# xingchensong/TouchNet

Hardware: AMD Instinct MI355X
Metric: audio+text tokens/sec/node (packed seq, full train step) + step MFU (higher is better)
Workload: dtype bf16

## Files before the change

touchnet_amd/_C.py:

```python
from __future__ import annotations

import ctypes as C
import os

import torch

_HERE = os.path.dirname(os.path.abspath(__file__))
LIB_PATH = os.environ.get("TN_AMD_LIB") or os.path.join(_HERE, "_lib", "libtouchnet_amd.so")

_vp, _i, _f, _ll, _ull = C.c_void_p, C.c_int, C.c_float, C.c_longlong, C.c_ulonglong

PROTOTYPES = {
    "tn_version": [],
    "tn_norm_bwd_workspace_floats": [_i, _i],
    "tn_rmsnorm_fwd": [_vp, _vp, _vp, _vp, _vp, _vp, _i, _i, _f, _i, _vp],
    "tn_rmsnorm_bwd": [_vp, _vp, _vp, _vp, _vp, _vp, _vp, _vp, _i, _i, _i, _vp],
    "tn_layernorm_fwd": [_vp, _vp, _vp, _vp, _vp, _vp, _vp, _vp, _i, _i, _f, _i, _vp],
    "tn_layernorm_bwd": [_vp, _vp, _vp, _vp, _vp, _vp, _vp, _vp, _vp, _vp, _i, _i, _i, _vp],
    "tn_swiglu_fwd": [_vp, _vp, _vp, _ll, _i, _vp],
    "tn_swiglu_bwd": [_vp, _vp, _vp, _vp, _vp, _ll, _i, _vp],
    "tn_gelu_fwd": [_vp, _vp, _ll, _i, _vp],
    "tn_gelu_bwd": [_vp, _vp, _vp, _ll, _i, _vp],
    "tn_rope_table": [_vp, _vp, _vp, _vp, _i, _i, _f, _i, _vp],
    "tn_rope_apply": [_vp, _vp, _vp, _vp, _vp, _vp, _i, _i, _i, _i, _i, _i, _vp],
# ... 36 lines not shown
    "tn_adamw_prepare": [_vp, _vp, _f, _f, _f, _vp],
    "tn_adamw_multi": [_vp, _vp, _vp, _vp, _vp, _vp, _vp, _i, _ll, _vp, _f, _f, _f, _f, _f, _i, _vp],
    "tn_adamw_multi_bounded": [_vp, _vp, _vp, _vp, _vp, _vp, _vp, _i, _ll, _vp, _f, _f, _f, _f, _f, _i, _i, _vp],
    "tn_pack_plan": [_vp, _i, _i, _i, _i, _vp, _vp, _vp, _vp, _vp, _vp],
    "tn_pack_fill": [_vp, _vp, _vp, _vp, _i, _i, _vp, _vp, _vp, _vp, _vp, _vp, _i, _i, _i, _ll, _ll, _ll, _vp, _vp, _vp,
                     _vp, _vp, _vp, _vp, _vp],
    "tn_gemm_bf16_tn": [_vp, _vp, _vp, _vp, _vp, _i, _i, _i, _ll, _ll, _ll, _ll, _i, _vp],
    "tn_gemm_bf16_addend": [_vp, _vp, _ll, _ll, _i, _i, _i, _vp, _vp, _vp, _ll, _i, _i, _ll, _vp],
    "tn_gemm_bf16_splitk": [_vp, _vp, _ll, _ll, _i, _i, _i, _vp, _vp, _i, _i, _ll, _i, _i, _i, _vp, _ll, _vp],
    "tn_gemm_bf16_wgrad_f32": [_vp, _vp, _ll, _ll, _i, _vp, _i, _i, _ll, _i, _i, _vp, _ll, _vp],
    "tn_gemm_bf16": [C.POINTER(_vp), C.POINTER(_vp), C.POINTER(_ll), C.POINTER(_ll), C.POINTER(_i), _i, _i, _i, _vp, _vp,
                     _vp, _i, _i, _ll, _ll, _i, _vp],
    "tn_gemm_splitk_workspace_bytes": [_i, _i, _i, _i, _i],
    "tn_gemm_grouped_workspace_bytes": [C.POINTER(_i), C.POINTER(_i), C.POINTER(_i), _i],
    "tn_gemm_bf16_grouped": [C.POINTER(_vp), C.POINTER(_vp), C.POINTER(_ll), C.POINTER(_ll), C.POINTER(_i), C.POINTER(_vp),
                             C.POINTER(_ll), C.POINTER(_i), C.POINTER(_i), _i, _i, _i, _i, _i, _vp, _ll, _vp],
    "tn_gemm_grouped_table_bytes": [_i],
    "tn_gemm_bf16_grouped_table": [C.POINTER(_vp), C.POINTER(_vp), C.POINTER(_ll), C.POINTER(_ll), C.POINTER(_i),
                                   C.POINTER(_vp), C.POINTER(_ll), C.POINTER(_i), C.POINTER(_i), C.POINTER(_vp), _i, _i, _i,
                                   _vp, _ll, _vp],
    "tn_gemm_bf16_wgrad_bias": [_vp, _vp, _ll, _ll, _i, _vp, _vp, _i, _i, _ll, _i, _i, _i, _vp, _ll, _vp],
    "tn_gemm_bf16_rope": [_vp, _vp, _vp, _vp, _vp, _vp, _i, _i, _i, _ll, _ll, _ll, _i, _vp],
    "tn_gemm_bf16_gelu_fwd": [_vp, _vp, _vp, _vp, _vp, _i, _i, _i, _ll, _ll, _ll, _vp],
    "tn_gemm_bf16_gelu_bwd": [_vp, _vp, _vp, _vp, _i, _i, _i, _ll, _ll, _ll, _vp],
    "tn_gemm_bf16_swiglu_fwd": [_vp, _vp, _vp, _vp, _vp, _vp, _i, _i, _i, _ll, _ll, _ll, _vp],
    "tn_gemm_bf16_swiglu_bwd": [_vp, _vp, _vp, _vp, _vp, _vp, _i, _i, _i, _ll, _ll, _ll, _vp],
    "tn_gemm_set_persistent": [_i],
    "tn_gemm_get_persistent": [],
    "tn_attn_decode_workspace_bytes": [_i, _i, _i, _i, _i],
    "tn_attn_decode": [_vp, _vp, _vp, _vp, _vp, _vp, _vp, _vp, _i, _i, _i, _i, _i, _f, _vp],
    "tn_greedy_step": [_vp, _vp, _vp, _vp, _vp, _vp, _i, _i, _i, _f, _i, _i, _i, _i, _vp],
    "tn_sample_step": [_vp, _vp, _vp, _vp, _vp, _vp, _vp, _vp, _vp, _i, _i, _i, _f, _i, _f, _i, _f, _ull, _vp, _i, _i, _i,
                       _vp],
    "tn_kimi_text_step": [_vp] * 11 + [_i, _i, _i, _i, _f, _i, _f, _i, _ull, _i, _i, _i, _i, _vp],
    "tn_attn_decode_beam": [_vp, _vp, _vp, _vp, _vp, _vp, _vp, _vp, _vp, _i, _i, _i, _i, _i, _f, _vp],
    "tn_beam_step_workspace_bytes": [_i, _i],
    "tn_beam_step": [_vp] * 17 + [_i, _i, _i, _i, _i, _f, _i, _vp, _i, _i, _f, _i, _i, _vp],
    "tn_logits_constrain": [_vp] * 13 + [_i] * 11 + [_vp],
    "tn_beam_step_edits": [_vp] * 17 + [_i, _i, _i, _i, _i, _f, _i, _vp, _i, _i, _f, _i, _i, _vp, _vp, _vp, _i, _vp],
    "tn_token_scores": [_vp] * 8 + [_i] * 5 + [_vp],
    "tn_attn_block_causal_fwd": [_vp, _vp, _vp, _vp, _vp, _vp, _i, _i, _i, _i, _i, _f, _vp],
    "tn_vq_nearest": [_vp, _vp, _vp, _vp, _i, _i, _i, _vp],
    "tn_edit_align_ws_words": [_i, _i],
    "tn_edit_align": [_vp, _ll, _vp, _ll, _vp, _vp, _i, _vp, _ll, _vp, _ll, _vp, _vp],
}
_RESTYPE = {"tn_gemm_set_persistent": None, "tn_version": C.c_char_p, "tn_sumsq_multi_chunk": C.c_longlong, "tn_adamw_multi_chunk": C.c_longlong,
            "tn_colsum_workspace_floats": C.c_longlong, "tn_gemm_splitk_workspace_bytes": C.c_longlong,
            "tn_gemm_grouped_workspace_bytes": C.c_longlong, "tn_gemm_grouped_table_bytes": C.c_longlong,
            "tn_attn_decode_workspace_bytes": C.c_longlong, "tn_beam_step_workspace_bytes": C.c_longlong,
            "tn_edit_align_ws_words": C.c_longlong, "tn_philox4x32_10": None}

DEV_PROTOTYPES = {
    "tn_philox4x32_10": [_vp, _ull],
}

_lib = None


class KernelError(RuntimeError):
    pass


def lib() -> C.CDLL:
    global _lib
    if _lib is None:
        if not os.path.exists(LIB_PATH):
            raise ImportError(
                f"{LIB_PATH} not found: build it with `python -m touchnet_amd.build` "
                "(touchnet_amd has no fallback path; the HIP extension is mandatory)")
        handle = C.CDLL(LIB_PATH)
        for name, argtypes in {**PROTOTYPES, **DEV_PROTOTYPES}.items():
            fn = getattr(handle, name)
            fn.argtypes = argtypes
            fn.restype = _RESTYPE.get(name, C.c_int)
        _lib = handle
    return _lib


def check(code: int, what: str) -> None:
    if code != 0:
        raise KernelError(f"{what} failed with code {code} "
                          f"({'EINVAL: unsupported shape/dtype' if code == -22 else 'hipError_t'})")


DTYPE_CODE = {torch.float32: 0, torch.bfloat16: 1}


def dcode(t: torch.Tensor) -> int:
    try:
        return DTYPE_CODE[t.dtype]
    except KeyError:
        raise KernelError(f"unsupported dtype {t.dtype} (float32 / bfloat16 only)") from None


def ptr(t):
    if t is None:
        return None
    if not t.is_cuda:
        raise KernelError("touchnet_amd kernels need device (HIP) tensors; got a CPU tensor")
    return C.c_void_p(t.data_ptr())


def stream():
    return C.c_void_p(torch.cuda.current_stream().cuda_stream)


# ... 3 lines not shown
```

touchnet_amd/csrc/gemm.hip:

```cpp
#include "gemm_host.h"

namespace tn {
namespace gemm {

typedef f32x4_t Acc16[8][4];

template <bool AK, bool BK, int EPI = EPI_PLAIN>
struct Kernel16 {
  static_assert(EPI == EPI_PLAIN || EPI == EPI_SWIGLU_FWD || EPI == EPI_SWIGLU_BWD || EPI == EPI_ROPE ||
                    EPI == EPI_GELU_FWD || EPI == EPI_GELU_BWD,
                "Kernel16: plain / SwiGLU / RoPE / GELU epilogues (the weight-gradient modes stay on Kernel)");
  static_assert(EPI != EPI_GELU_FWD || !BK, "GELU forward: x W^T layout");
  static_assert(EPI != EPI_GELU_BWD || BK, "GELU backward: dY W layout");
  static_assert(!AK, "Kernel16: row-stored A (forward and input-gradient products)");
  static_assert(EPI != EPI_SWIGLU_FWD || !BK, "SwiGLU forward: x W^T layout");
  static_assert(EPI != EPI_SWIGLU_BWD || BK, "SwiGLU backward: dY W layout");
  static_assert(EPI != EPI_ROPE || !BK, "RoPE epilogue: x W^T layout");
  static constexpr int BN_EFF = EPI == EPI_SWIGLU_FWD ? 128 : BN;
  static __device__ __forceinline__ float sigm(float x) { return sigmoid_fast(x); }
  static __device__ __forceinline__ float lo16(uint32_t w) { return __uint_as_float(w << 16); }
  static __device__ __forceinline__ float hi16(uint32_t w) { return __uint_as_float(w & 0xffff0000u); }
  static __device__ __forceinline__ float rbf(float v) { return __uint_as_float(((uint32_t)f2bf(v)) << 16); }
  template <bool KMAJ>
  struct F4 {
// ... 1 lines not shown
    u32x2_t h[KMAJ ? 4 : 1][2];
  };
  template <bool KMAJ, int NB >
  struct Reader {
    int x[KMAJ ? NB / 2 : 2];
    __device__ __forceinline__ Reader(int lane, int row0) {
      const int l15 = lane & 15, g4 = lane >> 4;
      if constexpr (!KMAJ) {
        const int f = (l15 >> 1) & 7;
#pragma unroll
        for (int h = 0; h < 2; ++h) x[h] = (row0 + l15) * 128 + (((4 * h + g4) ^ f) << 4);
      } else {
        const int j = l15 >> 2, w = l15 & 3;
#pragma unroll
        for (int g = 0; g < NB / 2; ++g)
          x[g] = (8 * g4 + j) * 512 + w * 8 + ((((row0 >> 5) + g) ^ j) << 6) + (g4 & 1) * 32;
      }
    }
    template <int H, int BLK, int I>
    __device__ __forceinline__ void read(const char* smem, int sbase, F4<KMAJ>& f) const {
      if constexpr (!KMAJ) {
        f.v[I] = __builtin_bit_cast(bf16x8_t, *reinterpret_cast<const u32x4_t*>(smem + sbase + x[H] + BLK * 2048));
      } else {
        const uint32_t a = (uint32_t)(size_t)(lds_ptr_t)smem + (uint32_t)(sbase + (x[BLK >> 1] ^ ((BLK & 1) * 32)));
        f.h[I][0] = ds_tr16<(32 * H) * 512>(a);
        f.h[I][1] = ds_tr16<(32 * H + 4) * 512>(a);
      }
    }
  };
  template <bool KMAJ>
  static __device__ __forceinline__ void retire(F4<KMAJ>& f) {
    if constexpr (KMAJ) {
      asm volatile("s_waitcnt lgkmcnt(0)"
                   : "+v"(f.h[0][0]), "+v"(f.h[0][1]), "+v"(f.h[1][0]), "+v"(f.h[1][1]), "+v"(f.h[2][0]), "+v"(f.h[2][1]),
                     "+v"(f.h[3][0]), "+v"(f.h[3][1]));
#pragma unroll
      for (int i = 0; i < 4; ++i) {
        const u32x4_t t = {f.h[i][0].x, f.h[i][0].y, f.h[i][1].x, f.h[i][1].y};
        f.v[i] = __builtin_bit_cast(bf16x8_t, t);
      }
    }
  }

  static __device__ __forceinline__ void run(const Params& p, char* smem) {
    const int tid = threadIdx.x;
    int lane = tid & 63;
    const int wave = __builtin_amdgcn_readfirstlane(tid >> 6);
    const int wr = wave >> 2, wc = wave & 3;
    const int bid = blockIdx.x, G = gridDim.x;
    const int tiles = p.ntiles;
    const int mine = (tiles - bid + G - 1) / G;
    auto origin = [&](int k, int& m0, int& n0) {
      int tm, tn;
      tile_of_block(p.tile0 + bid + k * G, p.nbm, p.nbn, tm, tn);
      m0 = tm * BM;
      n0 = tn * BN_EFF;
    };
    Stream<AK, true> sA;
    Stream<BK, true> sB;
    int ka = 0, kb = 0;
    auto open_a = [&](int s) {
      int m0, n0;
      origin(ka, m0, n0);
      sA.open(p.seg[s].A, p.seg[s].lda, p.seg[s].K, p.M, m0, wave, lane);
      sA.seg = s;
    };
    const bool b_wave0 = EPI == EPI_SWIGLU_FWD || (EPI == EPI_ROPE && p.rope_d == 128);
    auto open_b = [&](int s) {
      int m0, n0;
      origin(kb, m0, n0);
      if constexpr (EPI == EPI_SWIGLU_FWD) {
        sB.open((wave & 1) ? p.seg[1].B : p.seg[0].B, p.seg[0].ldb, p.seg[0].K, p.N, n0 + (wave >> 1) * 32, 0, lane);
      } else if constexpr (EPI == EPI_ROPE) {
        if (p.rope_d == 128)
          sB.open(p.seg[0].B, p.seg[0].ldb, p.seg[0].K, p.N, n0 + (wave >> 2) * 128 + (wave & 1) * 64 + ((wave >> 1) & 1) * 32,
                  0, lane);
        else
          sB.open(p.seg[0].B, p.seg[0].ldb, p.seg[0].K, p.N, n0, wave, lane);
      } else {
        sB.open(p.seg[s].B, p.seg[s].ldb, p.seg[s].K, p.N, n0, wave, lane);
      }
      sB.seg = s;
    };
    auto adv_a = [&]() {
      sA.soff += sA.step;
      if (--sA.left == 0) {
        if (sA.seg + 1 < p.nseg) open_a(sA.seg + 1);
        else if (++ka < mine) open_a(0);
        else sA.kill(p.C);
      }
    };
    auto adv_b = [&]() {
      sB.soff += sB.step;
      if (--sB.left == 0) {
        if (sB.seg + 1 < p.nseg) open_b(sB.seg + 1);
        else if (++kb < mine) open_b(0);
        else sB.kill(p.C);
      }
    };
    auto piece_a = [&](int slot, int q) {
      __builtin_amdgcn_raw_ptr_buffer_load_lds(sA.rs, (lds_ptr_t)(smem + slot * SLOT + wave * 4096 + q * 1024), 16,
                                               sA.voff[q], sA.soff, 0, 0);
    };
    auto piece_b = [&](int slot, int q) {
      __builtin_amdgcn_raw_ptr_buffer_load_lds(sB.rs, (lds_ptr_t)(smem + slot * SLOT + wave * 4096 + q * 1024), 16,
                                               sB.voff[q], sB.soff, 0, 0);
    };
// ... 629 lines not shown
  if (c.addend != nullptr && (c.accumulate || c.splitk > 1 || c.tail_only || c.Ct != nullptr || c.c_f32 ||
                              c.bias_grad != nullptr || !out_ok(c.addend, c.ldadd, N, 8)))
    return TN_EINVAL;
  if ((c.bias_grad != nullptr || c.c_f32) && (!wgrad_mode || c.tail_only)) return TN_EINVAL;
  if (!aligned(1, c.bias_grad)) return TN_EINVAL;
  if (M <= 0 || N <= 0 || c.nseg < 1 || c.nseg > MAXSEG || (N % 8) != 0 || (c.a_kmaj && (M % 8))) return TN_EINVAL;
  if (!out_ok(c.C, c.ldc, N, 8)) return TN_EINVAL;
  if (c.Ct != nullptr && ((M % 8) || c.accumulate || !out_ok(c.Ct, c.ldct, M, 8))) return TN_EINVAL;
  Params p;
  clear_params(p);
  for (int s = 0; s < c.nseg; ++s) {
    const int k = c.K[s];
    if (!(c.a_kmaj ? kmaj_operand_ok(c.A[s], c.lda[s], k, M, M) : row_operand_ok(c.A[s], c.lda[s], k, 1))) return TN_EINVAL;
    if (!(c.b_kmaj ? kmaj_operand_ok(c.B[s], c.ldb[s], k, N, 1) : row_operand_ok(c.B[s], c.ldb[s], k, 1))) return TN_EINVAL;
    set_seg(p.seg[s], c.A[s], c.B[s], c.lda[s], c.ldb[s], k);
    p.stages += (k + 63) / 64;
  }
  for (int s = c.nseg; s < MAXSEG; ++s) p.seg[s] = p.seg[0];
  p.nseg = c.nseg;
  p.M = M;
  p.N = N;
  p.C = (bf16_t*)c.C;
  p.Ct = (bf16_t*)c.Ct;
  p.bias = (const bf16_t*)c.bias;
  p.ldc = c.ldc;
  p.ldct = c.ldct;
  p.accumulate = c.accumulate;
  p.addend = (const bf16_t*)c.addend;
  p.ldadd = c.ldadd;
  p.nbm = (M + BM - 1) / BM;
  p.nbn = (N + BN - 1) / BN;
  p.ntiles = p.nbm * p.nbn;
  p.c_f32 = c.c_f32;
  p.bias_out = (bf16_t*)c.bias_grad;
  const int ncu = num_cus();
  int main_tiles = 0;
  if (c.splitk > 1) {
    if (c.nseg != 1 || c.Ct != nullptr) return TN_EINVAL;
    if (!(c.a_kmaj && c.b_kmaj) && (p.stages % c.splitk) != 0) return TN_EINVAL;
    const long long need = tn_gemm_splitk_workspace_bytes(M, N, c.splitk, c.bias_grad != nullptr, c.tail_only);
    if (need < 0 || c.workspace == nullptr || !aligned(15, c.workspace) || c.workspace_bytes < need) return TN_EINVAL;
    if (c.tail_only) main_tiles = p.ntiles / ncu * ncu;
    p.splitk = c.splitk;
    p.kchunk = (p.stages + c.splitk - 1) / c.splitk;
    p.ws = (float*)c.workspace;
    if (c.bias_grad != nullptr) p.bias_ws = p.ws + slab_floats(c.splitk, p.ntiles);
  }
  hipStream_t st = (hipStream_t)c.stream;
  int rc = 0;
  if (main_tiles > 0) {
    Params pm = p;
    pm.splitk = 1;
    pm.ntiles = main_tiles;
    rc |= launch_mode(c.a_kmaj, c.b_kmaj, c.Ct != nullptr, dim3(ncu), st, pm);
    p.tile0 = main_tiles;
    p.ntiles -= main_tiles;
  }
  rc |= launch_mode(c.a_kmaj, c.b_kmaj, c.Ct != nullptr, grid_for(p.ntiles * p.splitk), st, p);
  if (rc != 0) return TN_EINVAL;
  TN_LAUNCH_CHECK();
  return TN_OK;
}

template <int EPI, bool B_KMAJ>
int launch_fused(Params& p, int M, int N, long long ldc, int col_tile, void* stream) {
  for (int s = 1; s < MAXSEG; ++s)
    if (p.seg[s].K == 0) p.seg[s] = p.seg[0];
  p.stages = p.seg[0].K / 64;
  p.M = M;
  p.N = N;
  p.ldc = ldc;
  p.nbm = (M + BM - 1) / BM;
  p.nbn = (N + col_tile - 1) / col_tile;
  p.ntiles = p.nbm * p.nbn;
  hipLaunchKernelGGL((gemm16_kernel<false, B_KMAJ, EPI>), grid_for(p.ntiles), dim3(NT), 0, (hipStream_t)stream, p);
  TN_LAUNCH_CHECK();
  return TN_OK;
}

}

extern "C" {

void tn_gemm_set_persistent(int on) { g_persistent = on ? 1 : 0; }
int tn_gemm_get_persistent(void) { return g_persistent; }

long long tn_gemm_splitk_workspace_bytes(int M, int N, int splitk, int with_bias_grad, int tail_only) {
  if (splitk <= 1) return 0;
  if (M <= 0 || N <= 0) return -1;
  const long long nbm = (M + BM - 1) / BM;
  long long tiles = nbm * ((N + BN - 1) / BN);
  if (tail_only) {
    const int ncu = num_cus();
    if (tiles < ncu || tiles % ncu == 0) return -1;
    tiles %= ncu;
  }
  return (slab_floats(splitk, tiles) + (with_bias_grad ? splitk * nbm * BM : 0)) * (long long)sizeof(float);
}

int tn_gemm_bf16(const void* const* A, const void* const* B, const long long* lda, const long long* ldb, const int* K,
                 int nseg, int a_kmaj, int b_kmaj, void* C, void* Ct, const void* bias, int M, int N, long long ldc,
                 long long ldct, int accumulate, void* stream) {
  GemmCall c{A, B, lda, ldb, K, nseg, a_kmaj, b_kmaj, C, ldc, M, N, stream};
  c.bias = bias;
  c.accumulate = accumulate;
  c.Ct = Ct;
  c.ldct = ldct;
  return gemm_launch(c);
}

int tn_gemm_bf16_addend(const void* A, const void* B, long long lda, long long ldb, int K, int a_kmaj, int b_kmaj, void* C,
                        const void* bias, const void* addend, long long ldadd, int M, int N, long long ldc, void* stream) {
  if (addend == nullptr || addend == C) return TN_EINVAL;
  GemmCall c{&A, &B, &lda, &ldb, &K, 1, a_kmaj, b_kmaj, C, ldc, M, N, stream};
  c.bias = bias;
  c.addend = addend;
  c.ldadd = ldadd;
  return gemm_launch(c);
}

int tn_gemm_bf16_splitk(const void* A, const void* B, long long lda, long long ldb, int K, int a_kmaj, int b_kmaj,
                        void* C, const void* bias, int M, int N, long long ldc, int accumulate, int splitk, int tail_only,
                        void* workspace, long long workspace_bytes, void* stream) {
  if (splitk < 2) return TN_EINVAL;
  GemmCall c{&A, &B, &lda, &ldb, &K, 1, a_kmaj, b_kmaj, C, ldc, M, N, stream};
  c.bias = bias;
  c.accumulate = accumulate;
  c.splitk = splitk;
  c.tail_only = tail_only;
  c.workspace = workspace;
  c.workspace_bytes = workspace_bytes;
  return gemm_launch(c);
}

static int wgrad(const void* A, const void* B, long long lda, long long ldb, int K, void* C, void* bias_grad, int M, int N,
                 long long ldc, int accumulate, int c_f32, int splitk, void* workspace, long long workspace_bytes,
                 void* stream) {
  GemmCall c{&A, &B, &lda, &ldb, &K, 1, 1, 1, C, ldc, M, N, stream};
// ... 12 lines not shown
  return wgrad(A, B, lda, ldb, K, C, nullptr, M, N, ldc, accumulate, 1, splitk, workspace, workspace_bytes, stream);
}

int tn_gemm_bf16_wgrad_bias(const void* A, const void* B, long long lda, long long ldb, int K, void* C, void* bias_grad,
                            int M, int N, long long ldc, int accumulate, int c_f32, int splitk, void* workspace,
                            long long workspace_bytes, void* stream) {
  if (bias_grad == nullptr) return TN_EINVAL;
  return wgrad(A, B, lda, ldb, K, C, bias_grad, M, N, ldc, accumulate, c_f32, splitk, workspace, workspace_bytes, stream);
}

long long tn_gemm_grouped_workspace_bytes(const int* M, const int* N, const int* K, int ngrp) {
  if (ngrp < 1 || ngrp > MAXSEG) return -1;
  long long tiles = 0;
  int min_stages = 0x7fffffff, r;
  for (int g = 0; g < ngrp; ++g) {
    tiles += (long long)((M[g] + BM - 1) / BM) * ((N[g] + BN - 1) / BN);
    min_stages = min(min_stages, (K[g] + 63) / 64);
  }
  const int S = grouped_split(tiles, min_stages, r);
  return S > 1 ? slab_floats(S, r) * (long long)sizeof(float) : 0;
}

int tn_gemm_bf16_grouped(const void* const* A, const void* const* B, const long long* lda, const long long* ldb,
                         const int* K, void* const* C, const long long* ldc, const int* M, const int* N, int ngrp,
                         int a_kmaj, int b_kmaj, int accumulate, int c_f32, void* workspace, long long workspace_bytes,
                         void* stream) {
  if (ngrp < 1 || ngrp > MAXSEG) return TN_EINVAL;
  if (!(a_kmaj && b_kmaj)) return TN_EINVAL;
  Params p;
  clear_params(p);
  int total = 0, min_stages = 0x7fffffff;
  for (int g = 0; g < ngrp; ++g) {
    if (!grouped_product(A[g], B[g], lda[g], ldb[g], K[g], C[g], ldc[g], M[g], N[g], c_f32, total, p.seg[g], p.grp[g]))
      return TN_EINVAL;
    min_stages = min(min_stages, p.grp[g].stages);
    total += p.grp[g].nbm * p.grp[g].nbn;
  }
  for (int g = ngrp; g < MAXSEG; ++g) {
    p.seg[g] = p.seg[0];
    p.grp[g] = p.grp[0];
    p.grp[g].start = 0x7fffffff;
  }
  p.ngrp = ngrp;
  p.accumulate = accumulate;
  p.c_f32 = c_f32;
  hipStream_t st = (hipStream_t)stream;
  int r, S = grouped_split(total, min_stages, r);
  if (S > 1 && (workspace == nullptr || !aligned(15, workspace) ||
                workspace_bytes < slab_floats(S, r) * (long long)sizeof(float)))
    S = 1;
  const int main_tiles = S > 1 ? total - r : total;
  p.tile0 = 0;
  p.ntiles = main_tiles;
  if (c_f32)
    hipLaunchKernelGGL((gemm_kernel<true, true, false, false, true, EPI_GROUPED>), grid_for(main_tiles), dim3(NT), 0, st, p);
  else
    hipLaunchKernelGGL((gemm_kernel<true, true, false, false, false, EPI_GROUPED>), grid_for(main_tiles), dim3(NT), 0, st, p);
  if (S > 1) {
    float* ws = (float*)workspace;
    for (int g = 0; g < ngrp; ++g) {
      const int end = p.grp[g].start + p.grp[g].nbm * p.grp[g].nbn;
      const int lo = max(main_tiles, p.grp[g].start), hi = end;
      if (lo >= hi) continue;
      Params q;
      clear_params(q);
      q.seg[0] = p.seg[g];
      q.seg[1] = q.seg[2] = q.seg[0];
      q.M = p.grp[g].M;
      q.N = p.grp[g].N;
      q.C = p.grp[g].C;
      q.ldc = p.grp[g].ldc;
      q.accumulate = accumulate;
      q.nbm = p.grp[g].nbm;
      q.nbn = p.grp[g].nbn;
      q.stages = p.grp[g].stages;
      q.splitk = S;
      q.kchunk = (q.stages + S - 1) / S;
      q.ws = ws;
      q.tile0 = lo - p.grp[g].start;
      q.ntiles = hi - lo;
      q.c_f32 = c_f32;
      hipLaunchKernelGGL((gemm_kernel<true, true, false, true>), grid_for(q.ntiles * S), dim3(NT), 0, st, q);
      hipLaunchKernelGGL(splitk_reduce_kernel, dim3((unsigned)q.ntiles * 32u), dim3(256), 0, st, q.ws, q.splitk, q.M, q.N,
                         q.nbm, q.nbn, q.tile0, q.ntiles, q.C, q.ldc, (const bf16_t*)nullptr, q.accumulate, q.c_f32,
                         (const float*)nullptr, (bf16_t*)nullptr);
      ws += slab_floats(S, q.ntiles);
    }
  }
  TN_LAUNCH_CHECK();
  return TN_OK;
}
int tn_gemm_bf16_swiglu_fwd(const void* x, const void* wg, const void* wu, void* gate, void* up, void* act, int M, int I,
                            int K, long long ldx, long long ldw, long long ldc, void* stream) {
  if (M <= 0 || I <= 0 || (I % 8) || !row_operand_ok(x, ldx, K, K) || !row_operand_ok(wg, ldw, K, K) ||
      !row_operand_ok(wu, ldw, K, K) || !out_ok(gate, ldc, I, 8) || !aligned(15, up, act))
    return TN_EINVAL;
  Params p;
  clear_params(p);
  set_seg(p.seg[0], x, wg, ldx, ldw, K);
  set_seg(p.seg[1], x, wu, ldx, ldw, K);
  p.C = (bf16_t*)gate;
  p.C2 = (bf16_t*)up;
  p.C3 = (bf16_t*)act;
  return launch_fused<EPI_SWIGLU_FWD, false>(p, M, I, ldc, 128, stream);
}

// ... 69 lines not shown
```

touchnet_amd/csrc/gemm_host.h:

```cpp
#pragma once

#include "gemm_kernel.h"

using namespace tn::gemm;
using tn::bf16_t;

extern "C" int tn_gemm_get_persistent(void);

namespace {

int num_cus() {
  static const int ncu = [] {
    int dev = 0, n = 256;
    if (hipGetDevice(&dev) == hipSuccess) (void)hipDeviceGetAttribute(&n, hipDeviceAttributeMultiprocessorCount, dev);
    return n >= 8 ? n / 8 * 8 : 8;
  }();
  return ncu;
}

bool persistent_now() {
  const char* pe = getenv("TN_GEMM_PERSIST");
  return pe ? atoi(pe) != 0 : tn_gemm_get_persistent() != 0;
}

dim3 grid_for(int units) {
  const int ncu = num_cus();
  return dim3(persistent_now() && units > ncu ? ncu : units);
}

void clear_params(Params& p) {
  p = Params{};
  p.splitk = 1;
  p.nseg = 1;
}

void set_seg(Seg& s, const void* A, const void* B, long long lda, long long ldb, int K) {
  s.A = (const bf16_t*)A;
  s.B = (const bf16_t*)B;
  s.lda = lda;
  s.ldb = ldb;
  s.K = K;
  s.pad_ = 0;
}

template <typename... P>
bool aligned(uintptr_t mask, P... ps) {
  return ((... | (uintptr_t)ps) & mask) == 0;
}

constexpr long long DMA_SPAN = 0x7fffffffLL;

bool row_operand_ok(const void* X, long long ld, int K, long long min_ld) {
  return K > 0 && (K % 64) == 0 && aligned(15, X) && (ld % 8) == 0 && ld >= min_ld && 288 * ld * 2 < DMA_SPAN;
}

bool kmaj_operand_ok(const void* X, long long ld, int K, int rows, long long min_ld) {
  return K > 0 && aligned(15, X) && (ld % 8) == 0 && ld >= min_ld && ((long long)(K - 1) * ld + rows) * 2 < DMA_SPAN;
}

bool out_ok(const void* C, long long ld, int cols, int ld_mult) { return aligned(15, C) && (ld % ld_mult) == 0 && ld >= cols; }

bool grouped_product(const void* A, const void* B, long long lda, long long ldb, int k, void* C, long long ldc, int m, int n,
                     int c_f32, int start, Seg& s, Grp& g) {
  if (m <= 0 || n <= 0 || (m % 8) || (n % 8) || !kmaj_operand_ok(A, lda, k, m, m) || !kmaj_operand_ok(B, ldb, k, n, 1) ||
      !out_ok(C, ldc, n, c_f32 ? 4 : 8))
    return false;
  set_seg(s, A, B, lda, ldb, k);
  g.C = (bf16_t*)C;
  g.ldc = ldc;
  g.M = m;
  g.N = n;
  g.nbm = (m + BM - 1) / BM;
  g.nbn = (n + BN - 1) / BN;
  g.start = start;
  g.stages = (k + 63) / 64;
  return true;
}

}
```

touchnet_amd/csrc/gemm_kernel.h:

```cpp
#pragma once

#include <stdlib.h>

#include <type_traits>
#include <utility>
#include <vector>

#include "common.h"

namespace tn {
namespace gemm {

constexpr int BM = 256, BN = 256;
constexpr int SLOT = 32768;
constexpr int LDS_BYTES = 5 * SLOT;
constexpr int NT = 512;
constexpr int MAXSEG = 3;

typedef __attribute__((address_space(3))) void* lds_ptr_t;
typedef __attribute__((ext_vector_type(2))) uint32_t u32x2_t;
typedef __attribute__((ext_vector_type(4))) uint32_t u32x4_t;

struct Seg {
  const bf16_t* A;
  const bf16_t* B;
  long long lda, ldb;
  int K;
  int pad_;
};

struct Grp {
  bf16_t* C;
  long long ldc;
  int M, N, nbm, nbn;
  int start;
  int stages;
};

struct Rec {
  Seg seg;
  Grp grp;
  bf16_t* bias_out;
};
typedef const __attribute__((address_space(4))) Rec* rec_ptr_t;
constexpr int MAXTAB = 1024;
constexpr int TABCHUNK = 32;

constexpr int EPI_PLAIN = 0, EPI_GROUPED = 1, EPI_SWIGLU_FWD = 2, EPI_SWIGLU_BWD = 3, EPI_BIASG = 4, EPI_ROPE = 5;
constexpr int EPI_GELU_FWD = 6, EPI_GELU_BWD = 7, EPI_TABLE = 8;

struct Params {
  Seg seg[MAXSEG];
  int nseg;
  int M, N;
  bf16_t* C;
  bf16_t* Ct;
  const bf16_t* bias;
  long long ldc, ldct;
  int accumulate;
  const bf16_t* addend;
  long long ldadd;
  int nbm, nbn;
  int stages;
  int splitk, kchunk;
  float* ws;
  int tile0, ntiles;
  int c_f32;
  Grp grp[MAXSEG];
  int ngrp;
  bf16_t* C2;
  bf16_t* C3;
  const bf16_t* E1;
  const bf16_t* E2;
  long long lde;
  bf16_t* bias_out;
  float* bias_ws;
  const bf16_t* rope_cos;
  const bf16_t* rope_sin;
  int rope_d;
  const Rec* table;
};

__device__ __forceinline__ int xcd_chunk(int bid, int total) {
  const int xcd = bid & 7, local = bid >> 3;
  const int q = total >> 3, r = total & 7;
  return (xcd < r ? xcd * (q + 1) : r * (q + 1) + (xcd - r) * q) + local;
}

__device__ __forceinline__ void panel_group(int vid, int nbm, int nbn, int& tm, int& tn) {
  constexpr int GM = 8;
  const int per_group = GM * nbn;
  const int g = vid / per_group, w = vid - g * per_group;
  const int gm = min(GM, nbm - g * GM);
  tm = g * GM + w % gm;
  tn = w / gm;
}

__device__ __forceinline__ void tile_of_block(int bid, int nbm, int nbn, int& tm, int& tn) {
  panel_group(xcd_chunk(bid, nbm * nbn), nbm, nbn, tm, tn);
}

typedef f32x16_t Acc[4][2];

constexpr int kPieceB[4] = {0, 2, 4, 6}, kPieceA[4] = {14, 18, 22, 26};
static_assert(kPieceB[3] < kPieceA[0], "every B piece is issued before the first A piece");

template <bool IS_A> constexpr int piece_at(int pos) {
  for (int i = 0; i < 4; ++i)
    if ((IS_A ? kPieceA[i] : kPieceB[i]) == pos) return i;
  return -1;
}
constexpr int early_piece_count() {
  int n = 0;
  for (int i = 0; i < 4; ++i) n += (kPieceB[i] < 8) + (kPieceA[i] < 8);
  return n;
}

template <bool KMAJ, bool M16 = false>
struct Stream {
  __amdgpu_buffer_rsrc_t rs;
  int soff;
  int step;
  int left;
  int seg;
  int ld2;
  int voff[4];

  __device__ __forceinline__ void set_voff(int wave, int lane) {
    if constexpr (!KMAJ) {
#pragma unroll
      for (int q = 0; q < 4; ++q) {
        const int row = wave * 32 + q * 8 + (lane >> 3);
        voff[q] = row * ld2 + (((lane & 7) ^ ((row >> 1) & 7)) << 4);
      }
    } else {
#pragma unroll
      for (int q = 0; q < 4; ++q) {
        const int k = wave * 8 + q * 2 + (lane >> 5);
        const int u = lane & 31;
        const int ch = M16 ? ((u & 3) ^ (((k >> 3) & 1) << 1)) : (u & 3);
        voff[q] = k * ld2 + ((((u >> 2) ^ (k & 3)) << 6) | (ch << 4));
      }
    }
  }

  __device__ __forceinline__ void open(const bf16_t* X, long long ld, int K, int R, int origin, int wave, int lane) {
    ld2 = (int)(ld * 2);
    if constexpr (!KMAJ) {
      const long long bytes = R > origin ? (long long)(R - origin - 1) * ld2 + 2LL * K : 0LL;
      rs = __builtin_amdgcn_make_buffer_rsrc((void*)(X + (long long)origin * ld), 0, (int)min(bytes, 0x7fffffffLL),
                                             0x00020000);
      step = 128;
    } else {
// ... 90 lines not shown
#pragma unroll
      for (int j = 0; j < 2; ++j) {
        const u32x4_t t = {b.h[j][0].x, b.h[j][0].y, b.h[j][1].x, b.h[j][1].y};
        b.v[j] = __builtin_bit_cast(bf16x8_t, t);
      }
    }
  }

  static __device__ __forceinline__ void run(const Params& p, char* smem) { body(p, smem); }

  static __device__ __forceinline__ void body(const Params& p, char* smem) {
    const int tid = threadIdx.x;
    int lane = tid & 63;
    const int wave = __builtin_amdgcn_readfirstlane(tid >> 6);
    const int wr = wave >> 2, wc = wave & 3;

    const int bid = blockIdx.x, G = gridDim.x;
    const int tiles = p.ntiles;
    const int mine = ((SPLITK ? tiles * p.splitk : tiles) - bid + G - 1) / G;
    const rec_ptr_t tab = (rec_ptr_t)p.table;
    auto seg_of = [&](int g) {
      if constexpr (EPI == EPI_TABLE) {
        Seg s;
        s.A = tab[g].seg.A;
        s.B = tab[g].seg.B;
        s.lda = tab[g].seg.lda;
        s.ldb = tab[g].seg.ldb;
        s.K = tab[g].seg.K;
        s.pad_ = 0;
        return s;
      } else {
        return p.seg[g];
      }
    };
    auto grp_of = [&](int g) {
      if constexpr (EPI == EPI_TABLE) {
        Grp r;
        r.C = tab[g].grp.C;
        r.ldc = tab[g].grp.ldc;
        r.M = tab[g].grp.M;
        r.N = tab[g].grp.N;
        r.nbm = tab[g].grp.nbm;
        r.nbn = tab[g].grp.nbn;
        r.start = tab[g].grp.start;
        r.stages = tab[g].grp.stages;
        return r;
      } else {
        return p.grp[g];
      }
    };
    auto origin_g = [&](int k, int& m0, int& n0, int& g) {
      int tm, tn, u = bid + k * G;
      if constexpr (SPLITK) u -= (u / tiles) * tiles;
      u += p.tile0;
      g = 0;
      if constexpr (EPI == EPI_TABLE) {
        u = xcd_chunk(u, tiles);
        int hi = p.ngrp - 1;
        while (g < hi) {
          const int mid = (g + hi + 1) >> 1;
          if (tab[mid].grp.start <= u) g = mid;
          else hi = mid - 1;
        }
      } else if constexpr (EPI == EPI_GROUPED) {
        if (p.ngrp > 1 && u >= p.grp[1].start) g = 1;
        if (p.ngrp > 2 && u >= p.grp[2].start) g = 2;
      }
      if constexpr (EPI == EPI_TABLE) {
        const Grp r = grp_of(g);
        panel_group(u - r.start, r.nbm, r.nbn, tm, tn);
      } else if constexpr (EPI == EPI_GROUPED) {
        const Grp r = grp_of(g);
        tile_of_block(u - r.start, r.nbm, r.nbn, tm, tn);
      } else {
        tile_of_block(u, p.nbm, p.nbn, tm, tn);
      }
      m0 = tm * BM;
      n0 = tn * BN;
    };
    auto origin = [&](int k, int& m0, int& n0) {
      int g;
      origin_g(k, m0, n0, g);
    };
    auto split_of = [&](int k) { return (bid + k * G) / tiles; };

    Stream<AK> sA;
    Stream<BK> sB;
    int ka = 0, kb = 0;
    auto open_a = [&](int s) {
      int m0, n0;
      origin(ka, m0, n0);
      if constexpr (SPLITK) {
        const int k0 = split_of(ka) * p.kchunk * 64, klen = min(p.seg[0].K - k0, p.kchunk * 64);
        if (klen > 0) sA.open(p.seg[0].A + (AK ? (long long)k0 * p.seg[0].lda : (long long)k0), p.seg[0].lda, klen, p.M,
                              m0, wave, lane);
        else sA.kill(p.C);
        sA.left = p.kchunk;
      } else if constexpr (MULTI) {
        int g;
        origin_g(ka, m0, n0, g);
        const Seg sg = seg_of(g);
        sA.open(sg.A, sg.lda, sg.K, grp_of(g).M, m0, wave, lane);
      } else {
        sA.open(p.seg[s].A, p.seg[s].lda, p.seg[s].K, p.M, m0, wave, lane);
      }
      sA.seg = s;
    };
    auto open_b = [&](int s) {
      int m0, n0;
      origin(kb, m0, n0);
      if constexpr (SPLITK) {
        const int k0 = split_of(kb) * p.kchunk * 64, klen = min(p.seg[0].K - k0, p.kchunk * 64);
        if (klen > 0) sB.open(p.seg[0].B + (BK ? (long long)k0 * p.seg[0].ldb : (long long)k0), p.seg[0].ldb, klen, p.N,
                              n0, wave, lane);
        else sB.kill(p.C);
        sB.left = p.kchunk;
      } else if constexpr (MULTI) {
        int g;
        origin_g(kb, m0, n0, g);
        const Seg sg = seg_of(g);
        sB.open(sg.B, sg.ldb, sg.K, grp_of(g).N, n0, wave, lane);
      } else {
        sB.open(p.seg[s].B, p.seg[s].ldb, p.seg[s].K, p.N, n0, wave, lane);
      }
      sB.seg = s;
    };
    auto adv_a = [&]() {
      sA.soff += sA.step;
// ... 397 lines not shown
```

touchnet_amd/csrc/gemm_table.hip:

```cpp
#include "gemm_host.h"

namespace tn {
namespace gemm {

struct RecChunk {
  Rec r[TABCHUNK];
};
static_assert(sizeof(Rec) % 8 == 0 && sizeof(RecChunk) <= 3072, "a chunk of records fits the kernel-argument segment");
constexpr int REC_WORDS = (int)(sizeof(Rec) / 8);

__global__ __launch_bounds__(TABCHUNK * REC_WORDS) void table_upload_kernel(const RecChunk c, Rec* dst, int n) {
  const int t = threadIdx.x;
  if (t < n * REC_WORDS)
    reinterpret_cast<unsigned long long*>(dst)[t] = reinterpret_cast<const unsigned long long*>(&c)[t];
}

}
}

extern "C" {

long long tn_gemm_grouped_table_bytes(int n) { return n < 1 || n > MAXTAB ? -1 : (long long)n * (long long)sizeof(Rec); }

int tn_gemm_bf16_grouped_table(const void* const* A, const void* const* B, const long long* lda, const long long* ldb,
                               const int* K, void* const* C, const long long* ldc, const int* M, const int* N,
                               void* const* bias_grad, int n, int accumulate, int c_f32, void* table, long long table_bytes,
                               void* stream) {
  if (n < 1 || n > MAXTAB) return TN_EINVAL;
  if (table == nullptr || !aligned(15, table) || table_bytes < tn_gemm_grouped_table_bytes(n)) return TN_EINVAL;
  std::vector<RecChunk> chunks((n + TABCHUNK - 1) / TABCHUNK);
  long long total = 0;
  for (int g = 0; g < n; ++g) {
    Rec& r = chunks[g / TABCHUNK].r[g % TABCHUNK];
    if (total > 0x7fffffff) return TN_EINVAL;
    if (!grouped_product(A[g], B[g], lda[g], ldb[g], K[g], C[g], ldc[g], M[g], N[g], c_f32, (int)total, r.seg, r.grp))
      return TN_EINVAL;
    r.bias_out = bias_grad != nullptr ? (bf16_t*)bias_grad[g] : nullptr;
    if (!aligned(1, r.bias_out)) return TN_EINVAL;
    total += (long long)r.grp.nbm * r.grp.nbn;
  }
  if (total > 0x7fffffff) return TN_EINVAL;
  hipStream_t st = (hipStream_t)stream;
  for (int c = 0; c * TABCHUNK < n; ++c)
    hipLaunchKernelGGL(table_upload_kernel, dim3(1), dim3(TABCHUNK * REC_WORDS), 0, st, chunks[c],
                       (Rec*)table + c * TABCHUNK, min(TABCHUNK, n - c * TABCHUNK));
  Params p;
  clear_params(p);
  p.table = (const Rec*)table;
  p.ngrp = n;
  p.accumulate = accumulate;
  p.c_f32 = c_f32;
  p.ntiles = (int)total;
  if (c_f32)
    hipLaunchKernelGGL((gemm_kernel<true, true, false, false, true, EPI_TABLE>), grid_for(p.ntiles), dim3(NT), 0, st, p);
  else
    hipLaunchKernelGGL((gemm_kernel<true, true, false, false, false, EPI_TABLE>), grid_for(p.ntiles), dim3(NT), 0, st, p);
  TN_LAUNCH_CHECK();
  return TN_OK;
}

}
```

Baseline: 23640.

## Add host-chosen window/serpentine tile order to improve per-XCD L2 panel reuse

Adds a tile-mapping module with a second ordering, round-based windows over CUs with serpentine column-strip walks. The host simulates panel fetches per XCD for both orders, picks the one with fewer distinct row/column panels, and caches the choice by shape. All GEMM kernels (plain, Kernel16, grouped, table) now map tile indices through this shared function. The aim is more A/B panel reuse within each XCD's L2. The cost is extra index arithmetic, including an inverse-mapping loop for partial launches, and a host-side mutex and map lookup on every launch.

```diff
diff --git a/touchnet_amd/_C.py b/touchnet_amd/_C.py
--- a/touchnet_amd/_C.py
+++ b/touchnet_amd/_C.py
@@ -112,6 +112,7 @@
 
 DEV_PROTOTYPES = {
     "tn_philox4x32_10": [_vp, _ull],
+    "tn_gemm_tilemap_units": [C.POINTER(_i), C.POINTER(_i), _i, _i, _i, _i, _i, _i, _i, _i, C.POINTER(_i)],
 }
 
 _lib = None
diff --git a/touchnet_amd/csrc/gemm.hip b/touchnet_amd/csrc/gemm.hip
--- a/touchnet_amd/csrc/gemm.hip
+++ b/touchnet_amd/csrc/gemm.hip
@@ -77,7 +77,8 @@
     const int mine = (tiles - bid + G - 1) / G;
     auto origin = [&](int k, int& m0, int& n0) {
       int tm, tn;
-      tile_of_block(p.tile0 + bid + k * G, p.nbm, p.nbn, tm, tn);
+      const tilemap::List L = {1, p.total, 0, tiles, p.round, p.order, 0};
+      tilemap::tile_of_unit(bid + k * G, L, p.nbm, p.nbn, tm, tn);
       m0 = tm * BM;
       n0 = tn * BN_EFF;
     };
@@ -813,10 +814,12 @@
     Params pm = p;
     pm.splitk = 1;
     pm.ntiles = main_tiles;
+    set_tile_order(pm, p.nbm * p.nbn);
     rc |= launch_mode(c.a_kmaj, c.b_kmaj, c.Ct != nullptr, dim3(ncu), st, pm);
     p.tile0 = main_tiles;
     p.ntiles -= main_tiles;
   }
+  if (p.splitk == 1) set_tile_order(p, p.ntiles);
   rc |= launch_mode(c.a_kmaj, c.b_kmaj, c.Ct != nullptr, grid_for(p.ntiles * p.splitk), st, p);
   if (rc != 0) return TN_EINVAL;
   TN_LAUNCH_CHECK();
@@ -834,6 +837,7 @@
   p.nbm = (M + BM - 1) / BM;
   p.nbn = (N + col_tile - 1) / col_tile;
   p.ntiles = p.nbm * p.nbn;
+  set_tile_order(p, p.ntiles);
   hipLaunchKernelGGL((gemm16_kernel<false, B_KMAJ, EPI>), grid_for(p.ntiles), dim3(NT), 0, (hipStream_t)stream, p);
   TN_LAUNCH_CHECK();
   return TN_OK;
@@ -845,6 +849,37 @@
 
 void tn_gemm_set_persistent(int on) { g_persistent = on ? 1 : 0; }
 int tn_gemm_get_persistent(void) { return g_persistent; }
+
+int tn_gemm_tilemap_units(const int* nbm, const int* nbn, int ngrp, int whole, int tile0, int ntiles, int round, int order,
+                          int unit0, int count, int* out) {
+  if (ngrp < 1 || nbm == nullptr || nbn == nullptr || out == nullptr) return TN_EINVAL;
+  std::vector<int> shapes, starts;
+  long long total = 0;
+  for (int g = 0; g < ngrp; ++g) {
+    if (nbm[g] < 1 || nbn[g] < 1) return TN_EINVAL;
+    starts.push_back((int)total);
+    shapes.insert(shapes.end(), {nbm[g], nbn[g]});
+    total += (long long)nbm[g] * nbn[g];
+    if (total > 0x7fffffff) return TN_EINVAL;
+  }
+  if (tile0 < 0 || ntiles < 1 || (long long)tile0 + ntiles > total || round < 8 || (round % 8) != 0) return TN_EINVAL;
+  if (whole && (tile0 != 0 || ntiles != total)) return TN_EINVAL;
+  if (unit0 < 0 || count < 0 || (long long)unit0 + count > ntiles) return TN_EINVAL;
+  if (order < 0) order = tile0 != 0 ? tilemap::ORDER_CHUNK : tile_order((int)total, ntiles, round, whole, shapes);
+  if ((order != tilemap::ORDER_CHUNK && order != tilemap::ORDER_WINDOW) || (order == tilemap::ORDER_WINDOW && tile0 != 0))
+    return TN_EINVAL;
+  const tilemap::List L = {ngrp, (int)total, tile0, ntiles, round, order, whole};
+  for (int i = 0; i < count; ++i)
+    tilemap::tile_of_unit(
+        unit0 + i, L, [&](int pos) { return tilemap::product_at(pos, ngrp, [&](int g) { return starts[g]; }); },
+        [&](int g) { return starts[g]; },
+        [&](int g, int& m, int& n) {
+          m = shapes[2 * g];
+          n = shapes[2 * g + 1];
+        },
+        out[3 * i], out[3 * i + 1], out[3 * i + 2]);
+  return order;
+}
 
 long long tn_gemm_splitk_workspace_bytes(int M, int N, int splitk, int with_bias_grad, int tail_only) {
   if (splitk <= 1) return 0;
@@ -963,6 +998,7 @@
   const int main_tiles = S > 1 ? total - r : total;
   p.tile0 = 0;
   p.ntiles = main_tiles;
+  set_tile_order(p, total);
   if (c_f32)
     hipLaunchKernelGGL((gemm_kernel<true, true, false, false, true, EPI_GROUPED>), grid_for(main_tiles), dim3(NT), 0, st, p);
   else
diff --git a/touchnet_amd/csrc/gemm_host.h b/touchnet_amd/csrc/gemm_host.h
--- a/touchnet_amd/csrc/gemm_host.h
+++ b/touchnet_amd/csrc/gemm_host.h
@@ -1,4 +1,8 @@
 #pragma once
+
+#include <map>
+#include <mutex>
+#include <vector>
 
 #include "gemm_kernel.h"
 
@@ -32,6 +36,40 @@
   p = Params{};
   p.splitk = 1;
   p.nseg = 1;
+}
+
+int tile_order(int total, int ntiles, int round, int whole, const std::vector<int>& shapes) {
+  if (whole) return tilemap::ORDER_CHUNK;
+  static std::mutex mu;
+  static std::map<std::vector<int>, int> known;
+  std::vector<int> key = {total, ntiles, round, whole};
+  key.insert(key.end(), shapes.begin(), shapes.end());
+  std::lock_guard<std::mutex> lock(mu);
+  auto it = known.find(key);
+  if (it != known.end()) return it->second;
+  const int n = (int)shapes.size() / 2;
+  std::vector<int> starts(n, 0);
+  for (int g = 1; g < n; ++g) starts[g] = starts[g - 1] + shapes[2 * g - 2] * shapes[2 * g - 1];
+  const tilemap::List L = {n, total, 0, ntiles, round, tilemap::ORDER_CHUNK, whole};
+  const int order = tilemap::choose_order(
+      L, [&](int g) { return starts[g]; },
+      [&](int g, int& nbm, int& nbn) {
+        nbm = shapes[2 * g];
+        nbn = shapes[2 * g + 1];
+      });
+  known.emplace(std::move(key), order);
+  return order;
+}
+
+void set_tile_order(Params& p, int total) {
+  std::vector<int> shapes;
+  if (p.ngrp > 0)
+    for (int g = 0; g < p.ngrp; ++g) shapes.insert(shapes.end(), {p.grp[g].nbm, p.grp[g].nbn});
+  else
+    shapes = {p.nbm, p.nbn};
+  p.total = total;
+  p.round = num_cus();
+  p.order = tile_order(total, p.ntiles, p.round, 0, shapes);
 }
 
 void set_seg(Seg& s, const void* A, const void* B, long long lda, long long ldb, int K) {
diff --git a/touchnet_amd/csrc/gemm_kernel.h b/touchnet_amd/csrc/gemm_kernel.h
--- a/touchnet_amd/csrc/gemm_kernel.h
+++ b/touchnet_amd/csrc/gemm_kernel.h
@@ -7,6 +7,7 @@
 #include <vector>
 
 #include "common.h"
+#include "gemm_tilemap.h"
 
 namespace tn {
 namespace gemm {
@@ -65,6 +66,7 @@
   int splitk, kchunk;
   float* ws;
   int tile0, ntiles;
+  int total, round, order;
   int c_f32;
   Grp grp[MAXSEG];
   int ngrp;
@@ -81,24 +83,7 @@
   const Rec* table;
 };
 
-__device__ __forceinline__ int xcd_chunk(int bid, int total) {
-  const int xcd = bid & 7, local = bid >> 3;
-  const int q = total >> 3, r = total & 7;
-  return (xcd < r ? xcd * (q + 1) : r * (q + 1) + (xcd - r) * q) + local;
-}
-
-__device__ __forceinline__ void panel_group(int vid, int nbm, int nbn, int& tm, int& tn) {
-  constexpr int GM = 8;
-  const int per_group = GM * nbn;
-  const int g = vid / per_group, w = vid - g * per_group;
-  const int gm = min(GM, nbm - g * GM);
-  tm = g * GM + w % gm;
-  tn = w / gm;
-}
-
-__device__ __forceinline__ void tile_of_block(int bid, int nbm, int nbn, int& tm, int& tn) {
-  panel_group(xcd_chunk(bid, nbm * nbn), nbm, nbn, tm, tn);
-}
+using tilemap::tile_of_block;
 
 typedef f32x16_t Acc[4][2];
 
@@ -295,28 +280,30 @@
     auto origin_g = [&](int k, int& m0, int& n0, int& g) {
       int tm, tn, u = bid + k * G;
       if constexpr (SPLITK) u -= (u / tiles) * tiles;
-      u += p.tile0;
-      g = 0;
+      const tilemap::List L = {MULTI ? p.ngrp : 1, EPI == EPI_TABLE ? tiles : p.total, p.tile0, tiles, p.round,
+                               SPLITK || EPI == EPI_TABLE ? tilemap::ORDER_CHUNK : p.order, EPI == EPI_TABLE};
       if constexpr (EPI == EPI_TABLE) {
-        u = xcd_chunk(u, tiles);
-        int hi = p.ngrp - 1;
-        while (g < hi) {
-          const int mid = (g + hi + 1) >> 1;
-          if (tab[mid].grp.start <= u) g = mid;
-          else hi = mid - 1;
-        }
+        auto start_of = [&](int i) { return tab[i].grp.start; };
+        tilemap::tile_of_unit(
+            u, L, [&](int pos) { return tilemap::product_at(pos, p.ngrp, start_of); }, start_of,
+            [&](int i, int& nbm, int& nbn) {
+              nbm = tab[i].grp.nbm;
+              nbn = tab[i].grp.nbn;
+            },
+            g, tm, tn);
       } else if constexpr (EPI == EPI_GROUPED) {
-        if (p.ngrp > 1 && u >= p.grp[1].start) g = 1;
-        if (p.ngrp > 2 && u >= p.grp[2].start) g = 2;
-      }
-      if constexpr (EPI == EPI_TABLE) {
-        const Grp r = grp_of(g);
-        panel_group(u - r.start, r.nbm, r.nbn, tm, tn);
-      } else if constexpr (EPI == EPI_GROUPED) {
-        const Grp r = grp_of(g);
-        tile_of_block(u - r.start, r.nbm, r.nbn, tm, tn);
-      } else {
-        tile_of_block(u, p.nbm, p.nbn, tm, tn);
+        auto pick = [&](int i, int Grp::*f) { return i == 0 ? p.grp[0].*f : i == 1 ? p.grp[1].*f : p.grp[2].*f; };
+        tilemap::tile_of_unit(
+            u, L, [&](int pos) { return (int)(p.ngrp > 1 && pos >= p.grp[1].start) + (int)(p.ngrp > 2 && pos >= p.grp[2].start); },
+            [&](int i) { return pick(i, &Grp::start); },
+            [&](int i, int& nbm, int& nbn) {
+              nbm = pick(i, &Grp::nbm);
+              nbn = pick(i, &Grp::nbn);
+            },
+            g, tm, tn);
+      } else {
+        g = 0;
+        tilemap::tile_of_unit(u, L, p.nbm, p.nbn, tm, tn);
       }
       m0 = tm * BM;
       n0 = tn * BN;
diff --git a/touchnet_amd/csrc/gemm_table.hip b/touchnet_amd/csrc/gemm_table.hip
--- a/touchnet_amd/csrc/gemm_table.hip
+++ b/touchnet_amd/csrc/gemm_table.hip
@@ -51,6 +51,9 @@
   p.accumulate = accumulate;
   p.c_f32 = c_f32;
   p.ntiles = (int)total;
+  p.total = p.ntiles;
+  p.round = num_cus();
+  p.order = tile_order(p.total, p.ntiles, p.round, 1, {});
   if (c_f32)
     hipLaunchKernelGGL((gemm_kernel<true, true, false, false, true, EPI_TABLE>), grid_for(p.ntiles), dim3(NT), 0, st, p);
   else
diff --git a/touchnet_amd/csrc/gemm_tilemap.h b/touchnet_amd/csrc/gemm_tilemap.h
--- /dev/null
+++ b/touchnet_amd/csrc/gemm_tilemap.h
@@ -0,0 +1,156 @@
+#pragma once
+
+#include <algorithm>
+#include <vector>
+
+namespace tn {
+namespace gemm {
+namespace tilemap {
+
+#define TN_TILEMAP_FN __host__ __device__ __forceinline__
+
+constexpr int ORDER_CHUNK = 0, ORDER_WINDOW = 1;
+constexpr int GM = 8;
+constexpr int SW = 4;
+
+struct List {
+  int ngrp;
+  int total;
+  int tile0;
+  int ntiles;
+  int round;
+  int order;
+  int whole;
+};
+
+TN_TILEMAP_FN int xcd_chunk(int bid, int total) {
+  const int xcd = bid & 7, local = bid >> 3;
+  const int q = total >> 3, r = total & 7;
+  return (xcd < r ? xcd * (q + 1) : r * (q + 1) + (xcd - r) * q) + local;
+}
+
+TN_TILEMAP_FN int xcd_chunk_inv(int pos, int total) {
+  const int q = total >> 3, r = total & 7;
+  const int b = r * (q + 1);
+  int xcd, local;
+  if (pos < b) {
+    xcd = pos / (q + 1);
+    local = pos - xcd * (q + 1);
+  } else {
+    xcd = (pos - b) / q;
+    local = pos - b - xcd * q;
+    xcd += r;
+  }
+  return local * 8 + xcd;
+}
+
+TN_TILEMAP_FN void panel_group(int vid, int nbm, int nbn, int& tm, int& tn) {
+  const int per_group = GM * nbn;
+  const int g = vid / per_group, w = vid - g * per_group;
+  const int gm = min(GM, nbm - g * GM);
+  tm = g * GM + w % gm;
+  tn = w / gm;
+}
+
+TN_TILEMAP_FN int panel_group_inv(int tm, int tn, int nbm, int nbn) {
+  const int g = tm / GM;
+  const int gm = min(GM, nbm - g * GM);
+  return g * GM * nbn + tn * gm + (tm - g * GM);
+}
+
+TN_TILEMAP_FN int window_pos(int u, int n, int round) {
+  const int base = u / round * round;
+  return base + xcd_chunk(u - base, min(round, n - base));
+}
+
+TN_TILEMAP_FN void strip_walk(int i, int nbm, int nbn, int& tm, int& tn) {
+  const int last = max(nbn / SW, 1) - 1;
+  const int per = SW * nbm;
+  const int s = min(i / per, last);
+  const int j = i - s * per;
+  const int w = s == last ? nbn - s * SW : SW;
+  const int row = j / w;
+  tm = (s & 1) ? nbm - 1 - row : row;
+  tn = s * SW + (j - row * w);
+}
+
+template <typename StartOf>
+TN_TILEMAP_FN int product_at(int pos, int ngrp, StartOf start_of) {
+  int g = 0, hi = ngrp - 1;
+  while (g < hi) {
+    const int mid = (g + hi + 1) >> 1;
+    if (start_of(mid) <= pos) g = mid;
+    else hi = mid - 1;
+  }
+  return g;
+}
+
+template <typename Find, typename StartOf, typename ShapeOf>
+TN_TILEMAP_FN void tile_of_unit(int u, const List& L, Find find, StartOf start_of, ShapeOf shape_of, int& g, int& tm,
+                                int& tn) {
+  int nbm, nbn;
+  if (L.order == ORDER_CHUNK) {
+    u += L.tile0;
+    if (L.whole) u = xcd_chunk(u, L.total);
+    g = find(u);
+    shape_of(g, nbm, nbn);
+    u -= start_of(g);
+    panel_group(L.whole ? u : xcd_chunk(u, nbm * nbn), nbm, nbn, tm, tn);
+    return;
+  }
+  for (;;) {
+    const int v = u < L.ntiles ? window_pos(u, L.ntiles, L.round) : u;
+    g = find(v);
+    shape_of(g, nbm, nbn);
+    strip_walk(v - start_of(g), nbm, nbn, tm, tn);
+    if (L.ntiles == L.total) return;
+    u = start_of(g) + xcd_chunk_inv(panel_group_inv(tm, tn, nbm, nbn), nbm * nbn);
+    if (u < L.ntiles) return;
+  }
+}
+
+TN_TILEMAP_FN void tile_of_unit(int u, const List& L, int nbm, int nbn, int& tm, int& tn) {
+  int g;
+  tile_of_unit(u, L, [](int) { return 0; }, [](int) { return 0; }, [&](int, int& m, int& n) { m = nbm; n = nbn; }, g, tm, tn);
+}
+
+TN_TILEMAP_FN void tile_of_block(int bid, int nbm, int nbn, int& tm, int& tn) {
+  panel_group(xcd_chunk(bid, nbm * nbn), nbm, nbn, tm, tn);
+}
+
+template <typename StartOf, typename ShapeOf>
+long long panel_fetches(const List& L, StartOf start_of, ShapeOf shape_of) {
+  long long n = 0;
+  std::vector<long long> rows, cols;
+  for (int base = 0; base < L.ntiles; base += L.round)
+    for (int x = 0; x < 8; ++x) {
+      rows.clear();
+      cols.clear();
+      for (int u = base + x; u < std::min(base + L.round, L.ntiles); u += 8) {
+        int g, tm, tn;
+        tile_of_unit(u, L, [&](int pos) { return product_at(pos, L.ngrp, start_of); }, start_of, shape_of, g, tm, tn);
+        rows.push_back(((long long)g << 32) | (unsigned)tm);
+        cols.push_back(((long long)g << 32) | (unsigned)tn);
+      }
+      for (auto* v : {&rows, &cols}) {
+        std::sort(v->begin(), v->end());
+        n += std::unique(v->begin(), v->end()) - v->begin();
+      }
+    }
+  return n;
+}
+
+template <typename StartOf, typename ShapeOf>
+int choose_order(List L, StartOf start_of, ShapeOf shape_of) {
+  if (L.tile0 != 0) return ORDER_CHUNK;
+  L.order = ORDER_CHUNK;
+  const long long chunk = panel_fetches(L, start_of, shape_of);
+  L.order = ORDER_WINDOW;
+  return panel_fetches(L, start_of, shape_of) < chunk ? ORDER_WINDOW : ORDER_CHUNK;
+}
+
+#undef TN_TILEMAP_FN
+
+}
+}
+}
```

Result: no change. 23730 (median of 6 runs) (+0.4%).
